# clayjohn/godot-volumetric-cloud-demo-v2

Hardware: AMD Instinct MI355X
Metric: Mrays/s + hemisphere fps, 2048x1024 @ 128x6 steps, 1/2/4/8 MI355X (higher is better)
Workload: dtype f32

## Files before the change

__graft_entry__.py:

```python
import os
import subprocess
import sys

ROOT = os.path.dirname(os.path.abspath(__file__))
PKG = os.path.join(ROOT, "godot-volumetric-cloud-demo-v2_amd")
if ROOT not in sys.path:
    sys.path.insert(0, ROOT)


def build():
    env = dict(os.environ)
    env.setdefault("PYTORCH_ROCM_ARCH", "gfx950")
    subprocess.check_call(["make", "-C", os.path.join(PKG, "csrc"), "-s", "ARCH=gfx950"], env=env)
    subprocess.check_call(["make", "-C", os.path.join(ROOT, "oracle"), "-s"])
    subprocess.check_call(["make", "-C", os.path.join(ROOT, "tests", "hostsim"), "-s"])
    subprocess.check_call(["make", "-C", os.path.join(ROOT, "tests", "satwalk"), "-s"])
    subprocess.check_call(["make", "-C", os.path.join(ROOT, "tests", "tilewalk"), "-s"])
    subprocess.check_call(["make", "-C", os.path.join(ROOT, "tests", "radiance_host"), "-s"])
    subprocess.check_call(["make", "-C", os.path.join(ROOT, "tests", "tlut_host"), "-s"])
    subprocess.check_call(["make", "-C", os.path.join(ROOT, "tests", "owners_host"), "-s"])
    subprocess.check_call(["make", "-C", os.path.join(ROOT, "tests", "lut_reuse_host"), "-s"])
    subprocess.check_call(["make", "-C", os.path.join(ROOT, "tests", "frame_ring_host"), "-s"])
    subprocess.check_call(["make", "-C", os.path.join(ROOT, "tests", "noise_set_host"), "-s"])
    subprocess.check_call(["make", "-C", os.path.join(ROOT, "tests", "mip_args_host"), "-s"])
    subprocess.check_call(["make", "-C", os.path.join(ROOT, "tests", "shadow_host"), "-s"])
    subprocess.check_call(["make", "-C", os.path.join(ROOT, "tests", "aerial_host"), "-s"])
    subprocess.check_call(["make", "-C", os.path.join(ROOT, "tests", "shafts_host"), "-s"])
    subprocess.check_call(["make", "-C", os.path.join(ROOT, "tests", "cloud_aerial_host"), "-s"])
    subprocess.check_call(["make", "-C", os.path.join(ROOT, "tests", "rays_host"), "-s"])
    subprocess.check_call(["make", "-C", os.path.join(ROOT, "gdext"), "-s"])
    subprocess.call(["make", "-C", os.path.join(PKG, "csrc"), "-s", "census", "ARCH=gfx950"], env=env)
    import gvcd_amd

    L = gvcd_amd.lib()
    assert L.csky_abi_version() == gvcd_amd._lib.ABI_VERSION
    if os.path.isdir("/root/reference/cloud_sky"):
        subprocess.check_call([sys.executable, os.path.join(ROOT, "oracle", "glsl_exec", "make_glsl_fixtures.py"), "--compile-only"], stdout=subprocess.DEVNULL)
    return None


def smoke():
    import numpy as np

    import gvcd_amd
# ... 52 lines not shown
```

godot-volumetric-cloud-demo-v2_amd/csrc/cloud_core.h:

```cpp
#pragma once
#include "csky_common.h"

namespace csky {

#if defined(__HIP_DEVICE_COMPILE__)
CSKY_HD float fast_rcp(float x) { return __builtin_amdgcn_rcpf(x); }
CSKY_HD float fast_exp2(float x) { return __builtin_amdgcn_exp2f(x); }
CSKY_HD float fast_log2(float x) { return __builtin_amdgcn_logf(x); }
#define CSKY_WAVE_ALL(x) (__all(x) != 0)
#else
CSKY_HD float fast_rcp(float x) { return 1.0f / x; }
CSKY_HD float fast_exp2(float x) { return exp2f(x); }
CSKY_HD float fast_log2(float x) { return log2f(x); }
#define CSKY_WAVE_ALL(x) (x)
#endif
CSKY_HD float fast_exp(float x) { return fast_exp2(x * 1.44269504088896f); }
CSKY_HD float fast_pow(float x, float y) { return fast_exp2(y * fast_log2(x)); }

#ifndef CSKY_PRIO_MATH
#define CSKY_PRIO_MATH 1
#endif
#if defined(__HIP_DEVICE_COMPILE__) && CSKY_PRIO_MATH > 0
#define CSKY_PRIO(n) __builtin_amdgcn_s_setprio(n)
#else
// ... 314 lines not shown
        const uint32_t sh2 = (uint32_t)(5 - lvl);
        const uint16_t* __restrict__ d = T.detail_lds + detail_level_offset(lvl);
        const uint32_t r00 = (((uint32_t)z0 << sh2) | (uint32_t)y0) << sh2, r10 = (((uint32_t)z0 << sh2) | (uint32_t)y1) << sh2;
        const uint32_t r01 = (((uint32_t)z1 << sh2) | (uint32_t)y0) << sh2, r11 = (((uint32_t)z1 << sh2) | (uint32_t)y1) << sh2;
        const uint32_t p00 = (uint32_t)d[r00 + x0] | ((uint32_t)d[r00 + x1] << 16), p10 = (uint32_t)d[r10 + x0] | ((uint32_t)d[r10 + x1] << 16);
        const uint32_t p01 = (uint32_t)d[r01 + x0] | ((uint32_t)d[r01 + x1] << 16), p11 = (uint32_t)d[r11 + x0] | ((uint32_t)d[r11 + x1] << 16);
        return lerpf(lerpf(lerp_h2(p00, ax), lerp_h2(p10, ax), ay), lerpf(lerp_h2(p01, ax), lerp_h2(p11, ax), ay), az) * (1.0f / (8.0f * 255.0f));
    }
    const uint32_t sh = (uint32_t)(5 - lvl), idx = detail_level_offset(lvl) + ((((((uint32_t)z0 << sh) | (uint32_t)y0) << sh)) | (uint32_t)x0);
    const uint4 q = *reinterpret_cast<const uint4*>(reinterpret_cast<const char*>(T.detail) + (idx << 4));
    return fmaf(az, fmaf(ay, lerp_h(q.w, ax), lerp_h(q.z, ax)), fmaf(ay, lerp_h(q.y, ax), lerp_h(q.x, ax))) * (1.0f / (8.0f * 255.0f));
}

CSKY_HD float height_fraction(float r) { return sat((r - SKY_B_RADIUS) * (1.0f / (SKY_T_RADIUS - SKY_B_RADIUS))); }

CSKY_HD float density_height_gradient(const FrameConsts& fc, float hf, float ct) {
    const float c = ct;
    constexpr float K = 1.0f / 255.0f;
    float gx, d1, gz, d2;
    if (fc.ct_mode == 1) {
        gx = 0.03f + c * (-0.02f * K); d1 = (0.3375f - 0.03f) + c * ((-0.275f + 0.02f) * K); gz = 0.18f + c * (0.6f * K); d2 = (0.25f - 0.18f) + c * ((0.75f - 0.6f) * K);
    } else if (fc.ct_mode == 2) {
        gx = 0.02f + c * 0.0f; d1 = (0.05f - 0.02f) + c * (0.3f * K); gz = 0.09f + c * (0.78f * K); d2 = (0.11f - 0.09f) + c * ((1.03f - 0.78f) * K);
    } else {
        const bool hi = ct >= 127.5f;
        gx = (hi ? 0.03f : 0.02f) + c * (hi ? -0.02f * K : 0.0f);
        d1 = (hi ? 0.3375f - 0.03f : 0.05f - 0.02f) + c * (hi ? (-0.275f + 0.02f) * K : 0.3f * K);
        gz = (hi ? 0.18f : 0.09f) + c * (hi ? 0.6f * K : 0.78f * K);
        d2 = (hi ? 0.25f - 0.18f : 0.11f - 0.09f) + c * (hi ? (0.75f - 0.6f) * K : (1.03f - 0.78f) * K);
    }
    const float r = fast_rcp(d1 * d2);
    const float t = sat((hf - gx) * (r * d2)) - sat((hf - gz) * (r * d1));
    return t * t * (3.0f - 2.0f * t);
}

template <class TS>
CSKY_HD float density(const TS& T, const FrameConsts& fc, float px, float py, float pz, float hf, float wr, float wb,
                      int lod_shape, int lod_detail) {
    const float wc = fc.cov255 * wb;
    const float g = density_height_gradient(fc, hf, wr);
    const float omw = 1.0f - wc;
    if (!(g > omw)) return 0.0f;
    float qx, qy, qz, sx, sy, sz;
    shape_coord(fc, px, py, pz, qx, qy, qz, sx, sy, sz);
#ifdef CSKY_BRICK_BOUND
    if (lod_shape == 0) {
        int bx, by, bz; float fx_, fy_, fz_;
        split_coord(sx * 128.0f - 0.5f, bx, fx_); split_coord(sy * 128.0f - 0.5f, by, fy_); split_coord(sz * 128.0f - 0.5f, bz, fz_);
        const uint32_t bi = ((((uint32_t)bz & 127u) >> 3) << 8) | ((((uint32_t)by & 127u) >> 3) << 4) | (((uint32_t)bx & 127u) >> 3);
        const float bm = T.brick[bi];
        if (!(bm * g > omw)) return 0.0f;
    }
#endif
    float nr, fbm;
    shape_tap(T, lod_shape, sx, sy, sz, nr, fbm);
// ... 2 lines not shown
    float num = (nr + omf) * g - omw * den1;
    if (!(num > 0.0f)) return 0.0f;
#ifdef CSKY_RESTORE_WC_FACTOR
    num = num * (wc * fast_rcp(1.0f - omw));
#endif
    detail_coord(fc, qx, qy, qz, sx, sy, sz);
    float hfbm = detail_tap(T, lod_detail, sx, sy, sz);
    CSKY_STAGE(3);
    const float k = sat(hf * 4.0f);
    hfbm = hfbm + k * (1.0f - 2.0f * hfbm);
    const float hm = hfbm * 0.4f * hf, den2 = 1.0f - hm;
    const float base = (num - hm * den1) * fast_rcp(den1 * den2);
    return fast_pow(sat(base), (1.0f - hf) * 0.8f + 0.5f);
}

template <class TS>
CSKY_HD float sample_density(const TS& T, const FrameConsts& fc, float px, float py, float pz, float hf, float wx, float wy,
                             int lod_shape, int lod_detail) {
    CSKY_STAGE(0);
    if (!(hf > fc.hf_lo && hf < fc.hf_hi)) return 0.0f;
    float wsx, wsy, wr, wb;
    weather_coord(px, pz, wx, wy, wsx, wsy);
    weather_tap_ts(T, wsx, wsy, wr, wb);
    CSKY_STAGE(1);
    return density(T, fc, px, py, pz, hf, wr, wb, lod_shape, lod_detail);
}

#if CSKY_SHAPE_POLY == 3
template <bool EAGER_DETAIL = true, bool SMALL_TABLE = false, class TS>
CSKY_HD float sample_density_eager(const TS& T, const FrameConsts& fc, float px, float py, float pz, float hf, float wx, float wy,
                                   int lod_shape, int lod_detail) {
    if constexpr (TS::cell32) return sample_density(T, fc, px, py, pz, hf, wx, wy, lod_shape, lod_detail);
    float d = 0.0f;
    if (hf > fc.hf_lo && hf < fc.hf_hi) {
        CSKY_PRIO(0);
        float wsx, wsy;
        weather_coord(px, pz, wx, wy, wsx, wsy);
        int wix, wiy; float wax, way;
        split_coord(wsx * 512.0f - 0.5f, wix, wax); split_coord(wsy * 512.0f - 0.5f, wiy, way);
        const uint4 wq = *reinterpret_cast<const uint4*>(reinterpret_cast<const char*>(T.weather) + (((((uint32_t)(wiy & 511)) << 9) | (uint32_t)(wix & 511)) << 4));
        float qx, qy, qz, sx, sy, sz;
        shape_coord(fc, px, py, pz, qx, qy, qz, sx, sy, sz);
        const int sn = SHAPE_N >> lod_shape, sm = sn - 1;
        const float sfn = pow2f(7 - lod_shape);
        int six, siy, siz; float sax, say, saz;
        split_coord(sx * sfn - 0.5f, six, sax); split_coord(sy * sfn - 0.5f, siy, say); split_coord(sz * sfn - 0.5f, siz, saz);
        const uint32_t ssh = (uint32_t)(7 - lod_shape);
        const uint32_t sidx = shape_level_offset(lod_shape) + shape_cell_offset((uint32_t)(six & sm), (uint32_t)(siy & sm), (uint32_t)(siz & sm), ssh);
        const uint4* __restrict__ sp = reinterpret_cast<const uint4*>(reinterpret_cast<const char*>(T.shape) + (sidx << 5));
        const uint4 tr = sp[0], tf = sp[1];
        float dsx, dsy, dsz;
        detail_coord(fc, qx, qy, qz, dsx, dsy, dsz);
        const bool tap = EAGER_DETAIL && lod_detail != 5;
        uint4 dq;
        float dax, day, daz;
        if (tap) {
            const int dn = DETAIL_N >> lod_detail, dm = dn - 1;
            const float dfn = pow2f(5 - lod_detail);
            int dix, diy, diz;
            split_coord(dsx * dfn - 0.5f, dix, dax); split_coord(dsy * dfn - 0.5f, diy, day); split_coord(dsz * dfn - 0.5f, diz, daz);
            const uint32_t dsh = (uint32_t)(5 - lod_detail);
            const uint32_t dlo = detail_level_offset(lod_detail), dcell = (((((uint32_t)(diz & dm)) << dsh) | (uint32_t)(diy & dm)) << dsh) | (uint32_t)(dix & dm);
            const uint32_t didx = dlo + dcell;
            if constexpr (SMALL_TABLE) {
                static_assert(TS::small_detail && EAGER_DETAIL, "the table belongs to the persistent form's light march");
                const uint32_t dfirst = lod_detail == TS::SMALL_DETAIL_FIRST ? 0u : detail_level_offset(TS::SMALL_DETAIL_FIRST + 1) - detail_level_offset(TS::SMALL_DETAIL_FIRST);
                const SmallDetailCell c = T.det_small[dfirst + dcell];
                dq.x = c.x; dq.y = c.y; dq.z = c.z; dq.w = c.w;
            } else {
                dq = *reinterpret_cast<const uint4*>(reinterpret_cast<const char*>(T.detail) + (didx << 4));
            }
        }
        CSKY_PRIO(CSKY_PRIO_MATH);
        const float wr = fmaf(way, lerp_h(wq.y, wax), lerp_h(wq.x, wax));
        const float wb = fmaf(way, lerp_h(wq.w, wax), lerp_h(wq.z, wax));
        const float wc = fc.cov255 * wb;
        const float g = density_height_gradient(fc, hf, wr);
        const float omw = 1.0f - wc;
        if (g > omw) {
            const float nr = fmaf(saz, fmaf(say, lerp_h(tr.w, sax), lerp_h(tr.z, sax)), fmaf(say, lerp_h(tr.y, sax), lerp_h(tr.x, sax))) * (1.0f / 255.0f);
            const float fbm = fmaf(saz, fmaf(say, lerp_h(tf.w, sax), lerp_h(tf.z, sax)), fmaf(say, lerp_h(tf.y, sax), lerp_h(tf.x, sax))) * (1.0f / (8.0f * 255.0f));
            const float omf = 1.0f - fbm, den1 = 1.0f + omf;
            float num = (nr + omf) * g - omw * den1;
            if (num > 0.0f) {
#ifdef CSKY_RESTORE_WC_FACTOR
                num = num * (wc * fast_rcp(1.0f - omw));
#endif
                float hfbm;
                if (tap) hfbm = fmaf(daz, fmaf(day, lerp_h(dq.w, dax), lerp_h(dq.z, dax)), fmaf(day, lerp_h(dq.y, dax), lerp_h(dq.x, dax))) * (1.0f / (8.0f * 255.0f));
                else if (EAGER_DETAIL) hfbm = T.detail_lod5;
                else hfbm = detail_tap(T, lod_detail, dsx, dsy, dsz);
                const float k = sat(hf * 4.0f);
                hfbm = hfbm + k * (1.0f - 2.0f * hfbm);
                const float hm = hfbm * 0.4f * hf, den2 = 1.0f - hm;
                const float base = (num - hm * den1) * fast_rcp(den1 * den2);
                d = fast_pow(sat(base), (1.0f - hf) * 0.8f + 0.5f);
            }
        }
    }
    return d;
}
#else
template <bool EAGER_DETAIL = true, bool SMALL_TABLE = false, class TS>
CSKY_HD float sample_density_eager(const TS& T, const FrameConsts& fc, float px, float py, float pz, float hf, float wx, float wy,
                                   int lod_shape, int lod_detail) {
    return sample_density(T, fc, px, py, pz, hf, wx, wy, lod_shape, lod_detail);
}
#endif

CSKY_HD float henyey_greenstein(float c, float g) {
    const float x = 1.0f + g * g - 2.0f * g * c;
    return 0.0795774715459f * (1.0f - g * g) / (x * sqrtf(x));
}

CSKY_HD void shade_terms(const FrameConsts& fc, float phase, float t, float hf, float dt, float cd, float& Dr, float& Dg, float& Db, float& q) {
    const float lss = (SKY_T_RADIUS - SKY_B_RADIUS) / 64.0f;
    const float nd = -fc.density;
    const float beers = fast_exp(nd * cd * lss * 3.0f);
    const float powder = 1.0f - beers * beers;
    const float bt = 2.0f * beers * powder;
    const float sm = hf * hf * (3.0f - 2.0f * hf);
// ... 89 lines not shown
```

godot-volumetric-cloud-demo-v2_amd/csrc/cloud_kernels.hip:

```cpp
#include <hip/hip_runtime.h>
#include "kernels.h"
#include "cloud_core.h"
#include "order_core.h"
#pragma clang fp contract(off)

namespace csky {

constexpr int QCAP = 96;
constexpr int QSTEPS = 48;
constexpr int Q_FLOATS = 5 * QCAP + 7 * QCAP + 3 * QSTEPS;

__device__ __forceinline__ void wave_lds_fence() {
    __builtin_amdgcn_fence(__ATOMIC_RELEASE, "wavefront");
    __builtin_amdgcn_wave_barrier();
    __builtin_amdgcn_fence(__ATOMIC_ACQUIRE, "wavefront");
}

__device__ __forceinline__ float ray_phase(const FrameConsts& fc, const Ray& ray) {
    float phase = 0.0f;
    if (ray.above) {
        const float ct = fc.ldir[0] * ray.dx + fc.ldir[1] * ray.dy + fc.ldir[2] * ray.dz;
        phase = fmaxf(fmaxf(henyey_greenstein(ct, 0.6f), henyey_greenstein(ct, fc.hg_g2)), henyey_greenstein(ct, -0.2f));
    }
    return phase;
// ... 93 lines not shown
            if (!__any(live)) break;
        }
    }
    o.r = Lr; o.g = Lg; o.b = Lb; o.a = sat(alpha); o.t = Tr;
    return o;
}

constexpr int CQ_CAP = 128;
constexpr int CQ_STEPS = 66;
constexpr int CQ_FLOATS = 5 * CQ_CAP + CQ_CAP / 4 + 3 * CQ_STEPS + 2 + 128 + 320;

#ifndef CSKY_EAGER_LIGHT
#define CSKY_EAGER_LIGHT 1
#endif
#if CSKY_EAGER_LIGHT
#define CSKY_LIGHT_SAMPLE sample_density_eager<true>
#else
#define CSKY_LIGHT_SAMPLE sample_density
#endif
#ifndef CSKY_EAGER_PRIMARY
#define CSKY_EAGER_PRIMARY 0
#endif
#if CSKY_EAGER_PRIMARY == 1
#define CSKY_PRIMARY_SAMPLE sample_density_eager<false>
#elif CSKY_EAGER_PRIMARY == 2
#define CSKY_PRIMARY_SAMPLE sample_density_eager<true>
#else
#define CSKY_PRIMARY_SAMPLE sample_density
#endif
template <class TS, class Late>
__device__ __forceinline__ void light_march_terms(const TS& T, const FrameConsts& fc, const int ls, const float nd, float ex, float ey, float ez, Late&& late,
                                                  float& Dr, float& Dg, float& Db, float& rq, float& dt) {
    float lx = ex, ly = ey, lz = ez, cd = 0.0f;
#if CSKY_EAGER_LIGHT
    constexpr int JS = TS::small_detail ? 3 : 6;
#else
    constexpr int JS = 6;
#endif
#pragma unroll 1
    for (int j = 0; j < JS; j++) {
        if (j >= ls) break;
        advance(lx, ly, lz, fc.linc[j][0], fc.linc[j][1], fc.linc[j][2]);
        const float lhf = height_fraction(length3_shell(lx, ly, lz));
        cd += CSKY_LIGHT_SAMPLE(T, fc, lx, ly, lz, lhf, fc.wpos_x, fc.wpos_y, j > 2 ? j - 2 : 0, j);
    }
#if CSKY_EAGER_LIGHT
    if constexpr (TS::small_detail) {
#pragma unroll 1
        for (int j = JS; j < 6; j++) {
            if (j >= ls) break;
            advance(lx, ly, lz, fc.linc[j][0], fc.linc[j][1], fc.linc[j][2]);
            const float lhf = height_fraction(length3_shell(lx, ly, lz));
            cd += sample_density_eager<true, true>(T, fc, lx, ly, lz, lhf, fc.wpos_x, fc.wpos_y, j - 2, j);
        }
    }
#endif
    {
        lx = ex; ly = ey; lz = ez;
        advance(lx, ly, lz, fc.ldist[0], fc.ldist[1], fc.ldist[2]);
        const float lhf = height_fraction(length3_shell(lx, ly, lz));
        const float ld = CSKY_LIGHT_SAMPLE(T, fc, lx, ly, lz, lhf, 0.0f, 0.0f, 3, 5);
        cd += fast_pow(ld, (1.0f - lhf) * 0.8f + 0.5f);
    }
    float et, ehf, ess, eph;
    late(et, ehf, ess, eph);
    dt = fast_exp(nd * et * ess);
    shade_terms(fc, eph, et, ehf, dt, cd, Dr, Dg, Db, rq);
}

template <bool WHOLE, bool TALLY, class TS>
__device__ __forceinline__ MarchOut march_compact(const TS& T, const FrameConsts& fc, Ray ray, float* __restrict__ q, int step_begin, int step_end) {
    constexpr bool SAT = WHOLE && !TS::cell32;
    constexpr bool DEAD = SAT && !TALLY;
    float* __restrict__ ev_px = q;
    float* __restrict__ ev_py = q + CQ_CAP;
    float* __restrict__ ev_pz = q + 2 * CQ_CAP;
    float* __restrict__ ev_t = q + 3 * CQ_CAP;
    float* __restrict__ ev_hf = q + 4 * CQ_CAP;
    unsigned char* __restrict__ ev_owner = reinterpret_cast<unsigned char*>(q + 5 * CQ_CAP);
    unsigned* __restrict__ st_lo = reinterpret_cast<unsigned*>(q + 5 * CQ_CAP + CQ_CAP / 4);
    unsigned* __restrict__ st_hi = st_lo + CQ_STEPS;
    unsigned* __restrict__ st_base = st_hi + CQ_STEPS;

    MarchOut o; o.r = o.g = o.b = o.a = 0.0f; o.t = 1.0f; o.incloud = 0;
    const int lane = threadIdx.x & 63;
// ... 10 lines not shown
    float* __restrict__ ray_ss = reinterpret_cast<float*>(tally + 2);
    float* __restrict__ ray_ph = ray_ss + 64;
    ray_ss[lane] = ray.ss; ray_ph[lane] = phase;
    float* __restrict__ acc = ray_ph + 64;
    acc[lane] = 1.0f; acc[64 + lane] = 0.0f; acc[128 + lane] = 0.0f; acc[192 + lane] = 0.0f; acc[256 + lane] = 0.0f;
    if (__builtin_amdgcn_ballot_w64(live) == 0ull) return o;
    for (int i = 0; i < step_begin; i++) advance(px, py, pz, ray.sx, ray.sy, ray.sz);
    int end = step_end;
    for (int i = step_begin;;) {
        if (i < end) {
            float t, hf;
            bool have = false, below_top = false;
            if (live) {
                advance(px, py, pz, ray.sx, ray.sy, ray.sz);
                hf = height_fraction(length3_shell(px, py, pz));
                t = CSKY_PRIMARY_SAMPLE(T, fc, px, py, pz, hf, fc.wpos_x, fc.wpos_y, 0, 0);
                have = t > 0.0f;
                below_top = !(hf >= fc.hf_hi);
            }
            if constexpr (SAT && TALLY) {
                skipped += (unsigned)__popcll(__builtin_amdgcn_ballot_w64(have && latched));
                have = have && !latched;
            }
            if ((i & 3) == 3 && __builtin_amdgcn_ballot_w64(below_top) == 0ull) end = i + 1;
            const unsigned long long m = __builtin_amdgcn_ballot_w64(have);
            if (m != 0ull) {
                const int slot = count + (int)__builtin_amdgcn_mbcnt_hi((unsigned)(m >> 32), __builtin_amdgcn_mbcnt_lo((unsigned)m, 0u));
                if (have) { ev_px[slot] = px; ev_py[slot] = py; ev_pz[slot] = pz; ev_t[slot] = t; ev_hf[slot] = hf; ev_owner[slot] = (unsigned char)lane; }
                if (lane == 0) { st_lo[cs] = (unsigned)m; st_hi[cs] = (unsigned)(m >> 32); st_base[cs] = (unsigned)count; }
                count += __popcll(m);
                cs++;
            }
            i++;
        }
        const bool last = i >= end;
        if (count == 0) { if (last) break; continue; }
        if (count < 64 && !last) continue;
        wave_lds_fence();
        const int n = count < 64 ? count : 64;
        unsigned long long carry = 0ull;
        if constexpr (TALLY) { if (lane == 0) tally[0] += (unsigned)n; }
        if (lane < n) {
            float Dr, Dg, Db, rq, dt;
            light_march_terms(T, fc, ls, nd, ev_px[lane], ev_py[lane], ev_pz[lane],
                              [&](float& et, float& ehf, float& ess, float& eph) { et = ev_t[lane]; ehf = ev_hf[lane]; const int ow = ev_owner[lane]; ess = ray_ss[ow]; eph = ray_ph[ow]; }, Dr, Dg, Db, rq, dt);
            ev_px[lane] = Dr; ev_py[lane] = Dg; ev_pz[lane] = Db; ev_t[lane] = rq; ev_hf[lane] = dt;
        }
        wave_lds_fence();
        float Tr = acc[lane], alpha = acc[64 + lane], Lr = acc[128 + lane], Lg = acc[192 + lane], Lb = acc[256 + lane];
        for (int s = 0; s < cs; s++) {
            const unsigned lo = (unsigned)__builtin_amdgcn_readfirstlane((int)st_lo[s]), hi = (unsigned)__builtin_amdgcn_readfirstlane((int)st_hi[s]);
            const bool mine = __builtin_amdgcn_inverse_ballot_w64(((unsigned long long)hi << 32) | lo);
            const int slot = (int)st_base[s] + (int)__builtin_amdgcn_mbcnt_hi(hi, __builtin_amdgcn_mbcnt_lo(lo, 0u));
            if (mine && slot < n) {
                composite_sample(ev_hf[slot], ev_t[slot], ev_px[slot], ev_py[slot], ev_pz[slot], Tr, alpha, Lr, Lg, Lb);
            }
            if (s == cs - 1) carry = __builtin_amdgcn_ballot_w64(mine && slot >= n);
        }
        if constexpr (DEAD) {
// ... 198 lines not shown
        store_pixel(out, G, pix.gx, pix.gy, pix.lr, o.r, o.g, o.b, o.a);
    }
    if (stats || wg_cost) {
        unsigned ic = o.incloud, ab = ray.above ? 1u : 0u;
        for (int off = 32; off > 0; off >>= 1) { ic += __shfl_down(ic, off); ab += __shfl_down(ab, off); }
        if (lane == 0) {
            if (stats) { atomicAdd(&stats[0], (unsigned long long)ic); atomicAdd(&stats[1], (unsigned long long)ab); }
            if (wg_cost) atomicAdd(&wg_cost[logical], ic + 16u * ab);
        }
    }
}

#ifndef CSKY_COMPACT_WAVES
#define CSKY_COMPACT_WAVES 7
#endif
template <int VARIANT, int SEG, class TS = TexSet, bool TALLY = true>
__device__ __forceinline__ void render_block(TS T, const FrameConsts* __restrict__ fcp, const RenderGeom& G, const uint32_t logical, const uint32_t rec,
                                             uint2* __restrict__ out, unsigned long long* __restrict__ stats, uint32_t* __restrict__ wg_cost, const int tile_of_wave = -1) {
    constexpr int BW = 32 / SEG;
    const int tiles_x = (G.tile_w + BW - 1) / BW;
    const int local_rows = G.n_bands * G.band_rows;
    const int slab = (int)logical / tiles_x, bx = (int)logical - slab * tiles_x;
    const int wave = threadIdx.x >> 6, lane = threadIdx.x & 63;
    const int tile = tile_of_wave >= 0 ? tile_of_wave : wave / SEG, seg = tile_of_wave >= 0 ? 0 : wave - tile * SEG;
    const int gx = bx * BW + tile * 8 + (lane & 7);
    const int lr = slab * 8 + (lane >> 3);
    const bool valid = gx < G.tile_w && lr < local_rows;
    const int band = lr / G.band_rows, rib = lr - band * G.band_rows;
    const int gy = (G.first_band + band * G.band_stride) * G.band_rows + rib;

    const FrameConsts& fc = *fcp;
    T.detail_lds = nullptr;
    Ray ray = ray_setup(fc, valid ? gx : 0, valid ? gy : 0);
    if (!valid) ray.above = false;
    MarchOut o;
    if constexpr (VARIANT == 0) {
        static_assert(SEG == 1, "the lock-step reference variant marches whole rays");
        o = march(T, fc, ray);
    } else {
        __shared__ float lds[4][VARIANT == 3 ? CQ_FLOATS : Q_FLOATS];
        const int s0 = (fc.primary_steps * seg) / SEG, s1 = (fc.primary_steps * (seg + 1)) / SEG;
        if constexpr (VARIANT == 3) o = march_compact<SEG == 1, TALLY>(T, fc, ray, &lds[wave][0], s0, s1);
        else o = march_queue(T, fc, ray, &lds[wave][0], s0, s1);
        if constexpr (SEG > 1) {
            __shared__ float comb[4][5][64];
            comb[wave][0][lane] = o.r; comb[wave][1][lane] = o.g; comb[wave][2][lane] = o.b; comb[wave][3][lane] = o.t; comb[wave][4][lane] = o.a;
            __syncthreads();
            if (seg == 0) {
                float Tr = o.t, na = 1.0f - o.a;
#pragma unroll
                for (int s = 1; s < SEG; s++) {
                    const int w = tile * SEG + s;
                    o.r += Tr * comb[w][0][lane]; o.g += Tr * comb[w][1][lane]; o.b += Tr * comb[w][2][lane];
                    Tr *= comb[w][3][lane]; na *= 1.0f - comb[w][4][lane];
                }
                o.a = sat(1.0f - na); o.t = Tr;
            }
// ... 10 lines not shown
            if (stats) { atomicAdd(&stats[0], (unsigned long long)ic); atomicAdd(&stats[1], (unsigned long long)ab); }
            if (wg_cost) atomicAdd(&wg_cost[logical], ic + 16u * ab);
        }
    }
    }
}

template <int VARIANT, int SEG, class TS = TexSet, bool TALLY = true>
__global__ __launch_bounds__(256, VARIANT == 3 ? CSKY_COMPACT_WAVES : 7) void clouds_kernel(TS T, const FrameConsts* __restrict__ fcp, RenderGeom G, const uint32_t* __restrict__ order,
                                                     uint2* __restrict__ out, unsigned long long* __restrict__ stats, uint32_t* __restrict__ wg_cost) {
    const uint32_t logical = order[blockIdx.x];
    if (logical == 0xffffffffu) return;
    render_block<VARIANT, SEG, TS, TALLY>(T, fcp, G, logical, blockIdx.x, out, stats, wg_cost);
}

template <int VARIANT, bool TALLY = true>
__global__ __launch_bounds__(256, VARIANT == 3 ? CSKY_COMPACT_WAVES : 7) void clouds_kernel_persistent(TexSet T, const FrameConsts* __restrict__ fcp, RenderGeom G,
        const uint32_t* __restrict__ order, const uint32_t n_items, uint32_t* __restrict__ heads, uint2* __restrict__ out, unsigned long long* __restrict__ stats,
        uint32_t* __restrict__ wg_cost) {
    unsigned xcc;
    asm volatile("s_getreg_b32 %0, hwreg(HW_REG_XCC_ID)" : "=s"(xcc));
    xcc &= 7u;
    __shared__ uint32_t ticket, slot_ready[2], slot_reads[2], slot_entry[2], slot_rec[2];
    if (threadIdx.x == 0) { ticket = 0; slot_ready[0] = slot_ready[1] = 0; slot_reads[0] = slot_reads[1] = 0; }
    static_assert(VARIANT == 3, "the persistent form exists for the compact march only: its light march is the one that reads the table");
    __shared__ __attribute__((aligned(16))) uint4 det_small[TexSetSmallDetail::SMALL_DETAIL_CELLS];
    if (threadIdx.x < (unsigned)TexSetSmallDetail::SMALL_DETAIL_CELLS) det_small[threadIdx.x] = T.detail[detail_level_offset(TexSetSmallDetail::SMALL_DETAIL_FIRST) + threadIdx.x];
    __syncthreads();
    const bool lane0 = (threadIdx.x & 63) == 0;
    for (;;) {
        uint32_t tv = 0;
// ... 28 lines not shown
            }
            logical = (uint32_t)__builtin_amdgcn_readfirstlane((int)slot_entry[sl]);
            rec = (uint32_t)__builtin_amdgcn_readfirstlane((int)slot_rec[sl]);
            if (lane0) __hip_atomic_fetch_add(&slot_reads[sl], 1u, __ATOMIC_RELEASE, __HIP_MEMORY_SCOPE_WORKGROUP);
        }
        if (logical == 0xfffffffeu) {
            if (lane0 && atomicAdd(&heads[8], 1u) == gridDim.x * 4u - 1u) {
                for (unsigned k = 0; k < 9u; k++) atomicExch(&heads[k], 0u);
            }
            return;
        }
        if (logical != 0xffffffffu) {
            TexSetSmallDetail Ts;
            static_cast<TexSet&>(Ts) = T;
            Ts.det_small = (SmallDetailTable)det_small;
            render_block<VARIANT, 1, TexSetSmallDetail, TALLY>(Ts, fcp, G, logical, rec, out, stats, wg_cost, tile);
        }
    }
}


__global__ __launch_bounds__(256) void lpt_hist_kernel(const uint32_t* __restrict__ cost, int n, int shift, uint32_t* __restrict__ hist) {
    const int i = blockIdx.x * 256 + threadIdx.x;
    if (i < n) atomicAdd(&hist[lpt_bucket(cost[i], shift)], 1u);
}
__global__ __launch_bounds__(LPT_BUCKETS) void lpt_scan_kernel(uint32_t* __restrict__ hist, uint32_t* __restrict__ offsets) {
    __shared__ uint32_t sh[LPT_BUCKETS];
    const int t = threadIdx.x;
    const uint32_t own = hist[t];
    hist[t] = 0u;
    sh[t] = own;
// ... 54 lines not shown
    const size_t i = (size_t)blockIdx.x * 256 + threadIdx.x;
    if (i < n) out[i] = sqrt_shell(in[i]);
}
hipError_t launch_sqrt_shell(const float* d_in, float* d_out, size_t n, hipStream_t s) {
    if (n == 0) return hipSuccess;
    sqrt_shell_kernel<<<(unsigned)((n + 255) / 256), 256, 0, s>>>(d_in, d_out, n);
    return hipGetLastError();
}

static const char* const kVariantNames[] = {"lockstep", "queue", "queue-lds", "compact"};
int cloud_resident_workgroups_per_cu() { return CSKY_COMPACT_WAVES; }
int cloud_variant_count() { return (int)(sizeof(kVariantNames) / sizeof(kVariantNames[0])); }
const char* cloud_variant_name(int v) { return (v >= 0 && v < cloud_variant_count()) ? kVariantNames[v] : nullptr; }

hipError_t launch_clouds(int variant, int seg, const TexSet& t, const FrameConsts* d_fc, const RenderGeom& g, const uint32_t* d_order, int grid,
                         uint2* d_out, unsigned long long* d_stats, uint32_t* d_wg_cost, hipStream_t s, uint32_t* d_heads, int resident, const TexSet32* t32, bool census_lean) {
    if (grid <= 0) return hipSuccess;
    const bool tally = (d_stats != nullptr || d_wg_cost != nullptr) && !census_lean;
    if (t32) {
        if (variant != 3 || seg != 1) return hipErrorInvalidValue;
        clouds_kernel<3, 1, TexSet32><<<grid, 256, 0, s>>>(*t32, d_fc, g, d_order, d_out, d_stats, d_wg_cost);
        return hipGetLastError();
    }
    if (d_heads && variant == 3 && seg == 1) {
        if (tally) clouds_kernel_persistent<3, true><<<grid < resident ? grid : resident, 256, 0, s>>>(t, d_fc, g, d_order, (uint32_t)grid, d_heads, d_out, d_stats, d_wg_cost);
        else clouds_kernel_persistent<3, false><<<grid < resident ? grid : resident, 256, 0, s>>>(t, d_fc, g, d_order, (uint32_t)grid, d_heads, d_out, d_stats, d_wg_cost);
        return hipGetLastError();
    }
    if (variant == 0 && seg == 1) clouds_kernel<0, 1><<<grid, 256, 0, s>>>(t, d_fc, g, d_order, d_out, d_stats, d_wg_cost);
    else if (variant == 1 && seg == 1) clouds_kernel<1, 1><<<grid, 256, 0, s>>>(t, d_fc, g, d_order, d_out, d_stats, d_wg_cost);
    else if (variant == 1 && seg == 2) clouds_kernel<1, 2><<<grid, 256, 0, s>>>(t, d_fc, g, d_order, d_out, d_stats, d_wg_cost);
    else if (variant == 1 && seg == 4) clouds_kernel<1, 4><<<grid, 256, 0, s>>>(t, d_fc, g, d_order, d_out, d_stats, d_wg_cost);
    else if (variant == 3 && seg == 1 && tally) clouds_kernel<3, 1, TexSet, true><<<grid, 256, 0, s>>>(t, d_fc, g, d_order, d_out, d_stats, d_wg_cost);
    else if (variant == 3 && seg == 1) clouds_kernel<3, 1, TexSet, false><<<grid, 256, 0, s>>>(t, d_fc, g, d_order, d_out, d_stats, d_wg_cost);
    else if (variant == 3 && seg == 2) clouds_kernel<3, 2><<<grid, 256, 0, s>>>(t, d_fc, g, d_order, d_out, d_stats, d_wg_cost);
    else if (variant == 3 && seg == 4) clouds_kernel<3, 4><<<grid, 256, 0, s>>>(t, d_fc, g, d_order, d_out, d_stats, d_wg_cost);
    else if ((variant == 1 || variant == 3) && seg == 5) {
        hipError_t e = hipFuncSetAttribute(reinterpret_cast<const void*>(&clouds_kernel_interleaved<0>), hipFuncAttributeMaxDynamicSharedMemorySize,
                                           (int)(IL_BLOCK_FLOATS * sizeof(float)));
        if (e != hipSuccess) return e;
        clouds_kernel_interleaved<0><<<grid, 256, IL_BLOCK_FLOATS * sizeof(float), s>>>(t, d_fc, g, d_order, d_out, d_stats, d_wg_cost);
// ... 57 lines not shown
```

godot-volumetric-cloud-demo-v2_amd/csrc/clouds_launch.cpp:

```cpp
#include <cstring>
#include "context.h"
#include "launch_policy.h"
#include "order_core.h"

namespace csky {

TexSet texset(const csky_ctx* c) {
    const NoiseSet& n = c->noise;
    TexSet t;
#ifdef CSKY_BRICK_BOUND
    t.brick = n.d_brick;
#endif
    t.shape = n.d_shape; t.detail = n.d_detail; t.weather = n.d_weather; t.sky = c->lut.cur_f(); t.sky_w = c->lut.aw; t.sky_h = c->lut.ah; t.detail_lod5 = n.st.detail_lod5(); t.detail_h = n.d_detail_h; t.detail_lds = nullptr;
    return t;
}

TexSet32 texset32(const csky_ctx* c) {
    TexSet32 t;
    static_cast<TexSet&>(t) = texset(c);
    t.shape32 = c->noise.d_shape32; t.detail32 = c->noise.d_detail32; t.weather32 = c->noise.d_weather32;
    return t;
}

namespace {

int ensure_order(csky_ctx* c, int slot, int mode, int tiles_x, int slabs, hipStream_t s) {
    const int grid = static_order_grid(mode, tiles_x, slabs);
    const OrderKey key = order_key(tiles_x, slabs, mode, grid);
    FrameSlot& f = c->ring.slot[slot];
    if (f.order_st.hit(f.order != nullptr, key)) return CSKY_OK;
    if (f.order.count() < (size_t)grid) { int rc; if ((rc = c->ring.grow_order_tables(c, (size_t)grid))) return rc; }
    HIPCHK(c, launch_static_order(mode, tiles_x, slabs, grid, f.order, s));
    f.order_st.written(key);
    return CSKY_OK;
}

int frame_setup(csky_ctx* c, const CloudParams& cp, hipStream_t s) {
    const ExactRejects rej = c->noise.st.rejects(cp.cloud_coverage, c->use_window);
    int f, rc; if ((rc = c->ring.next_slot(c, c->stream, f))) return rc;
    const SetupArgs sa = {c->primary_steps, c->light_steps, c->early_eps, rej.hf_lo, rej.hf_hi, rej.ct_mode, c->use_window ? 1 : 0};
    const SkyLut& l = c->lut;
    if (l.st.own_taps())
        HIPCHK(c, launch_frame_setup_taps(cp, l.st.sun, c->d_trans_f, c->tw, c->th, l.st.w, l.st.h, sa, c->ring.slot[f].fc, c->stream, c->tlut));
    else
        HIPCHK(c, launch_frame_setup(cp, l.cur_f(), l.aw, l.ah, sa, c->ring.slot[f].fc, c->stream));
    return c->ring.setup_enqueued(c, f, c->stream, s);
}

}

int check_bands(csky_ctx* c, const csky_bands* b, int tile_w) {
    if (tile_w < 1 || !b || b->band_rows < 1 || b->n_bands < 0 || b->first_band < 0 || b->band_stride < 1)
        return fail(c, CSKY_ERR_INVALID, "render_clouds: bad tile/bands description");
    return CSKY_OK;
}
// ... 21 lines not shown
    if (c->noise.st.cell32()) { t32 = texset32(c); t32p = &t32; }
    const Event* kt = nullptr;
    if (c->kt.on && (rc = c->kt.next_pair(c, kt))) return rc;
    if ((rc = ensure_order(c, slot, pl.static_mode, tiles_x, slabs, s))) return rc;
    const uint32_t* order = ring.slot[slot].order;
    int grid = ring.slot[slot].order_st.grid();
    uint32_t* cost = nullptr;
    if (pl.feedback) {
        if ((rc = ring.reserve_feedback(c, (size_t)(grid > nblocks ? grid : nblocks)))) return rc;
        cost = ring.cost(slot);
        const FeedbackKey fkey = feedback_key(g.tile_w, g.band_rows, g.first_band, g.band_stride, g.n_bands, cp.texture_size, cp.update_position, pl.mode, pl.static_mode, pl.seg);
        if (ring.slot[slot].feedback.begin(fkey)) { order = ring.feedback_order(slot); grid = nblocks; }
    }
    if (kt) HIPCHK(c, hipEventRecord(kt[0], s));
    {
        const hipError_t le = launch_clouds(pl.variant, pl.seg, texset(c), ring.fc(), g, order, grid, d_out, d_stats, cost, s, heads, c->resident_wgs, t32p, c->census_lean);
        if (le != hipSuccess) { if (heads) (void)hipMemsetAsync(heads, 0, 16 * sizeof(uint32_t), s); return fail(c, CSKY_ERR_HIP, "cloud kernel launch failed: %s", hipGetErrorString(le)); }
    }
    if (kt) HIPCHK(c, hipEventRecord(kt[1], s));
    if (pl.feedback) {
        HIPCHK(c, launch_lpt_order(cost, nblocks, lpt_shift(c->primary_steps), ring.sort_scratch(slot), ring.feedback_order(slot), s));
        ring.slot[slot].feedback.sort_enqueued();
    }
    return ring.march_enqueued(c, slot, s);
}

}
```

godot-volumetric-cloud-demo-v2_amd/csrc/kernels.h:

```cpp
#pragma once
#include <hip/hip_runtime_api.h>
#include "csky_common.h"
#include "composite_core.h"
#include "noise_core.h"

namespace csky {

hipError_t launch_transmittance(int w, int h, uint16_t* d_half, float4* d_float, hipStream_t s, int tlut = 0);
hipError_t launch_sky_lut(int w, int h, const float sun[3], const float4* d_trans, int tw, int th, uint16_t* d_half,
                          float4* d_float, hipStream_t s, int tlut = 0);
hipError_t launch_sky_lut_rows(int w, int h, int row0, int row_stride, const float sun[3], const float4* d_trans, int tw, int th, uint2* d_rows, float4* d_whole_f,
                               hipStream_t s, int tlut = 0);
hipError_t launch_composite(const CompositeArgs& a, uint2* d_out, hipStream_t s, int tlut = 0);
struct SetupArgs {
    int primary_steps, light_steps;
    float early_eps, hf_lo, hf_hi;
    int ct_mode, sat_skip;
};
hipError_t launch_frame_setup(const CloudParams& p, const float4* d_sky, int sw, int sh, const SetupArgs& a, FrameConsts* d_fc, hipStream_t s);
hipError_t launch_frame_setup_taps(const CloudParams& p, const float sun[3], const float4* d_trans, int tw, int th, int sw, int sh, const SetupArgs& a, FrameConsts* d_fc,
                                   hipStream_t s, int tlut = 0);

hipError_t launch_shape_noise(uint32_t seed, int n, const ShapeNoiseParams& P, uint32_t* d_out, hipStream_t s);
hipError_t launch_detail_noise(uint32_t seed, int n, uint8_t* d_out, hipStream_t s);
hipError_t launch_mip_chain(uint8_t* d_chain, int n, int ch, int levels, hipStream_t s);
hipError_t launch_bake(const uint8_t* d_large_chain, const uint8_t* d_small_chain, const uint8_t* d_weather, ShapeTexel* d_shape, uint4* d_detail, uint16_t* d_detail_h,
                       uint4* d_weather_out, unsigned long long* d_inexact, int* d_range, hipStream_t s);
hipError_t launch_bake32(const uint8_t* d_large_chain, const uint8_t* d_small_chain, const uint8_t* d_weather, float4* d_shape32, float4* d_detail32, float4* d_weather32, hipStream_t s);

hipError_t launch_clouds(int variant, int seg, const TexSet& t, const FrameConsts* d_fc, const RenderGeom& g, const uint32_t* d_order, int grid,
                         uint2* d_out, unsigned long long* d_stats, uint32_t* d_wg_cost, hipStream_t s, uint32_t* d_heads = nullptr, int resident = 0,
                         const TexSet32* t32 = nullptr, bool census_lean = false);
int cloud_resident_workgroups_per_cu();
int cloud_variant_count();
const char* cloud_variant_name(int v);
hipError_t launch_lpt_order(uint32_t* d_cost, int n, int shift, uint32_t* d_scratch, uint32_t* d_order, hipStream_t s);
hipError_t launch_static_order(int mode, int tiles_x, int slabs, int grid, uint32_t* d_order, hipStream_t s);
hipError_t launch_interleave_bands(const void* d_gathered, size_t member_stride_bytes, int members, size_t band_bytes, int total_bands, void* d_frame, hipStream_t s);
hipError_t launch_sqrt_shell(const float* d_in, float* d_out, size_t n, hipStream_t s);
struct RaysGeom;
hipError_t launch_clouds_rays(const TexSet& t, const TexSet32* t32, const FrameConsts* d_fc, const RaysGeom& g, const float* d_dirs, uint2* d_out, hipStream_t s);

struct ShadowConsts;
hipError_t launch_cloud_shadow(const TexSet& t, const TexSet32* t32, const FrameConsts& fc, const ShadowConsts& sc, uint16_t* d_out, hipStream_t s);

struct AerialGeom;
hipError_t launch_aerial(const AerialGeom& g, const float4* d_trans, int tw, int th, uint2* d_out, hipStream_t s, int tlut = 0);
// ... 21 lines not shown
```

Measured before the change: 1582.

## Specialize persistent cloud kernel on cloud-type mode and straighten light march

Result: faster. 1640, median of 6 (+3.7%).

```diff
diff --git a/__graft_entry__.py b/__graft_entry__.py
--- a/__graft_entry__.py
+++ b/__graft_entry__.py
@@ -28,6 +28,7 @@
     subprocess.check_call(["make", "-C", os.path.join(ROOT, "tests", "shafts_host"), "-s"])
     subprocess.check_call(["make", "-C", os.path.join(ROOT, "tests", "cloud_aerial_host"), "-s"])
     subprocess.check_call(["make", "-C", os.path.join(ROOT, "tests", "rays_host"), "-s"])
+    subprocess.check_call(["make", "-C", os.path.join(ROOT, "tests", "gradient_host"), "-s"])
     subprocess.check_call(["make", "-C", os.path.join(ROOT, "gdext"), "-s"])
     subprocess.call(["make", "-C", os.path.join(PKG, "csrc"), "-s", "census", "ARCH=gfx950"], env=env)
     import gvcd_amd
diff --git a/godot-volumetric-cloud-demo-v2_amd/csrc/cloud_core.h b/godot-volumetric-cloud-demo-v2_amd/csrc/cloud_core.h
--- a/godot-volumetric-cloud-demo-v2_amd/csrc/cloud_core.h
+++ b/godot-volumetric-cloud-demo-v2_amd/csrc/cloud_core.h
@@ -352,13 +352,15 @@
 
 CSKY_HD float height_fraction(float r) { return sat((r - SKY_B_RADIUS) * (1.0f / (SKY_T_RADIUS - SKY_B_RADIUS))); }
 
+template <int CT = 0>
 CSKY_HD float density_height_gradient(const FrameConsts& fc, float hf, float ct) {
+    static_assert(CT >= 0 && CT <= 2, "cloud-type mode: 0 generic, 1 every texel >= 0.5, 2 every texel < 0.5");
     const float c = ct;
     constexpr float K = 1.0f / 255.0f;
     float gx, d1, gz, d2;
-    if (fc.ct_mode == 1) {
+    if (CT == 1 || (CT == 0 && fc.ct_mode == 1)) {
         gx = 0.03f + c * (-0.02f * K); d1 = (0.3375f - 0.03f) + c * ((-0.275f + 0.02f) * K); gz = 0.18f + c * (0.6f * K); d2 = (0.25f - 0.18f) + c * ((0.75f - 0.6f) * K);
-    } else if (fc.ct_mode == 2) {
+    } else if (CT == 2 || (CT == 0 && fc.ct_mode == 2)) {
         gx = 0.02f + c * 0.0f; d1 = (0.05f - 0.02f) + c * (0.3f * K); gz = 0.09f + c * (0.78f * K); d2 = (0.11f - 0.09f) + c * ((1.03f - 0.78f) * K);
     } else {
         const bool hi = ct >= 127.5f;
@@ -372,11 +374,11 @@
     return t * t * (3.0f - 2.0f * t);
 }
 
-template <class TS>
+template <int CT = 0, class TS>
 CSKY_HD float density(const TS& T, const FrameConsts& fc, float px, float py, float pz, float hf, float wr, float wb,
                       int lod_shape, int lod_detail) {
     const float wc = fc.cov255 * wb;
-    const float g = density_height_gradient(fc, hf, wr);
+    const float g = density_height_gradient<CT>(fc, hf, wr);
     const float omw = 1.0f - wc;
     if (!(g > omw)) return 0.0f;
     float qx, qy, qz, sx, sy, sz;
@@ -409,7 +411,7 @@
     return fast_pow(sat(base), (1.0f - hf) * 0.8f + 0.5f);
 }
 
-template <class TS>
+template <int CT = 0, class TS>
 CSKY_HD float sample_density(const TS& T, const FrameConsts& fc, float px, float py, float pz, float hf, float wx, float wy,
                              int lod_shape, int lod_detail) {
     CSKY_STAGE(0);
@@ -418,14 +420,20 @@
     weather_coord(px, pz, wx, wy, wsx, wsy);
     weather_tap_ts(T, wsx, wsy, wr, wb);
     CSKY_STAGE(1);
-    return density(T, fc, px, py, pz, hf, wr, wb, lod_shape, lod_detail);
+    return density<CT>(T, fc, px, py, pz, hf, wr, wb, lod_shape, lod_detail);
 }
 
 #if CSKY_SHAPE_POLY == 3
-template <bool EAGER_DETAIL = true, bool SMALL_TABLE = false, class TS>
+CSKY_HD uint32_t level_offset_scalar(uint32_t off) {
+#if defined(__HIP_DEVICE_COMPILE__)
+    asm("" : "+s"(off));
+#endif
+    return off;
+}
+template <bool EAGER_DETAIL = true, bool SMALL_TABLE = false, int CT = 0, class TS>
 CSKY_HD float sample_density_eager(const TS& T, const FrameConsts& fc, float px, float py, float pz, float hf, float wx, float wy,
                                    int lod_shape, int lod_detail) {
-    if constexpr (TS::cell32) return sample_density(T, fc, px, py, pz, hf, wx, wy, lod_shape, lod_detail);
+    if constexpr (TS::cell32) return sample_density<CT>(T, fc, px, py, pz, hf, wx, wy, lod_shape, lod_detail);
     float d = 0.0f;
     if (hf > fc.hf_lo && hf < fc.hf_hi) {
         CSKY_PRIO(0);
@@ -441,7 +449,8 @@
         int six, siy, siz; float sax, say, saz;
         split_coord(sx * sfn - 0.5f, six, sax); split_coord(sy * sfn - 0.5f, siy, say); split_coord(sz * sfn - 0.5f, siz, saz);
         const uint32_t ssh = (uint32_t)(7 - lod_shape);
-        const uint32_t sidx = shape_level_offset(lod_shape) + shape_cell_offset((uint32_t)(six & sm), (uint32_t)(siy & sm), (uint32_t)(siz & sm), ssh);
+        const uint32_t slo = CT != 0 ? level_offset_scalar(shape_level_offset(lod_shape)) : shape_level_offset(lod_shape);
+        const uint32_t sidx = slo + shape_cell_offset((uint32_t)(six & sm), (uint32_t)(siy & sm), (uint32_t)(siz & sm), ssh);
         const uint4* __restrict__ sp = reinterpret_cast<const uint4*>(reinterpret_cast<const char*>(T.shape) + (sidx << 5));
         const uint4 tr = sp[0], tf = sp[1];
         float dsx, dsy, dsz;
@@ -455,7 +464,7 @@
             int dix, diy, diz;
             split_coord(dsx * dfn - 0.5f, dix, dax); split_coord(dsy * dfn - 0.5f, diy, day); split_coord(dsz * dfn - 0.5f, diz, daz);
             const uint32_t dsh = (uint32_t)(5 - lod_detail);
-            const uint32_t dlo = detail_level_offset(lod_detail), dcell = (((((uint32_t)(diz & dm)) << dsh) | (uint32_t)(diy & dm)) << dsh) | (uint32_t)(dix & dm);
+            const uint32_t dlo = (CT != 0 && !SMALL_TABLE) ? level_offset_scalar(detail_level_offset(lod_detail)) : detail_level_offset(lod_detail), dcell = (((((uint32_t)(diz & dm)) << dsh) | (uint32_t)(diy & dm)) << dsh) | (uint32_t)(dix & dm);
             const uint32_t didx = dlo + dcell;
             if constexpr (SMALL_TABLE) {
                 static_assert(TS::small_detail && EAGER_DETAIL, "the table belongs to the persistent form's light march");
@@ -470,7 +479,7 @@
         const float wr = fmaf(way, lerp_h(wq.y, wax), lerp_h(wq.x, wax));
         const float wb = fmaf(way, lerp_h(wq.w, wax), lerp_h(wq.z, wax));
         const float wc = fc.cov255 * wb;
-        const float g = density_height_gradient(fc, hf, wr);
+        const float g = density_height_gradient<CT>(fc, hf, wr);
         const float omw = 1.0f - wc;
         if (g > omw) {
             const float nr = fmaf(saz, fmaf(say, lerp_h(tr.w, sax), lerp_h(tr.z, sax)), fmaf(say, lerp_h(tr.y, sax), lerp_h(tr.x, sax))) * (1.0f / 255.0f);
@@ -496,10 +505,10 @@
     return d;
 }
 #else
-template <bool EAGER_DETAIL = true, bool SMALL_TABLE = false, class TS>
+template <bool EAGER_DETAIL = true, bool SMALL_TABLE = false, int CT = 0, class TS>
 CSKY_HD float sample_density_eager(const TS& T, const FrameConsts& fc, float px, float py, float pz, float hf, float wx, float wy,
                                    int lod_shape, int lod_detail) {
-    return sample_density(T, fc, px, py, pz, hf, wx, wy, lod_shape, lod_detail);
+    return sample_density<CT>(T, fc, px, py, pz, hf, wx, wy, lod_shape, lod_detail);
 }
 #endif
 
diff --git a/godot-volumetric-cloud-demo-v2_amd/csrc/cloud_kernels.hip b/godot-volumetric-cloud-demo-v2_amd/csrc/cloud_kernels.hip
--- a/godot-volumetric-cloud-demo-v2_amd/csrc/cloud_kernels.hip
+++ b/godot-volumetric-cloud-demo-v2_amd/csrc/cloud_kernels.hip
@@ -2,6 +2,7 @@
 #include "kernels.h"
 #include "cloud_core.h"
 #include "order_core.h"
+#include <type_traits>
 #pragma clang fp contract(off)
 
 namespace csky {
@@ -131,44 +132,65 @@
 #define CSKY_EAGER_LIGHT 1
 #endif
 #if CSKY_EAGER_LIGHT
-#define CSKY_LIGHT_SAMPLE sample_density_eager<true>
+#define CSKY_LIGHT_SAMPLE(CT) sample_density_eager<true, false, CT>
 #else
-#define CSKY_LIGHT_SAMPLE sample_density
+#define CSKY_LIGHT_SAMPLE(CT) sample_density<CT>
 #endif
 #ifndef CSKY_EAGER_PRIMARY
 #define CSKY_EAGER_PRIMARY 0
 #endif
 #if CSKY_EAGER_PRIMARY == 1
-#define CSKY_PRIMARY_SAMPLE sample_density_eager<false>
+#define CSKY_PRIMARY_SAMPLE(CT) sample_density_eager<false, false, CT>
 #elif CSKY_EAGER_PRIMARY == 2
-#define CSKY_PRIMARY_SAMPLE sample_density_eager<true>
+#define CSKY_PRIMARY_SAMPLE(CT) sample_density_eager<true, false, CT>
 #else
-#define CSKY_PRIMARY_SAMPLE sample_density
+#define CSKY_PRIMARY_SAMPLE(CT) sample_density<CT>
 #endif
-template <class TS, class Late>
+#ifndef CSKY_LIGHT_STRAIGHT
+#define CSKY_LIGHT_STRAIGHT 1
+#endif
+#if CSKY_EAGER_LIGHT
+template <int CT, int J, class TS>
+__device__ __forceinline__ void light_samples_from(const TS& T, const FrameConsts& fc, const int ls, float& lx, float& ly, float& lz, float& cd) {
+    if constexpr (J < 6) {
+        if (J >= ls) return;
+        advance(lx, ly, lz, fc.linc[J][0], fc.linc[J][1], fc.linc[J][2]);
+        const float lhf = height_fraction(length3_shell(lx, ly, lz));
+        cd += sample_density_eager<true, (J > 2), CT>(T, fc, lx, ly, lz, lhf, fc.wpos_x, fc.wpos_y, J > 2 ? J - 2 : 0, J);
+        light_samples_from<CT, J + 1>(T, fc, ls, lx, ly, lz, cd);
+    }
+}
+#endif
+template <int CT = 0, class TS, class Late>
 __device__ __forceinline__ void light_march_terms(const TS& T, const FrameConsts& fc, const int ls, const float nd, float ex, float ey, float ez, Late&& late,
                                                   float& Dr, float& Dg, float& Db, float& rq, float& dt) {
     float lx = ex, ly = ey, lz = ez, cd = 0.0f;
 #if CSKY_EAGER_LIGHT
     constexpr int JS = TS::small_detail ? 3 : 6;
+    constexpr bool STRAIGHT = CSKY_LIGHT_STRAIGHT && TS::small_detail && CT != 0;
 #else
     constexpr int JS = 6;
+    constexpr bool STRAIGHT = false;
 #endif
+    if constexpr (!STRAIGHT) {
 #pragma unroll 1
-    for (int j = 0; j < JS; j++) {
-        if (j >= ls) break;
-        advance(lx, ly, lz, fc.linc[j][0], fc.linc[j][1], fc.linc[j][2]);
-        const float lhf = height_fraction(length3_shell(lx, ly, lz));
-        cd += CSKY_LIGHT_SAMPLE(T, fc, lx, ly, lz, lhf, fc.wpos_x, fc.wpos_y, j > 2 ? j - 2 : 0, j);
+        for (int j = 0; j < JS; j++) {
+            if (j >= ls) break;
+            advance(lx, ly, lz, fc.linc[j][0], fc.linc[j][1], fc.linc[j][2]);
+            const float lhf = height_fraction(length3_shell(lx, ly, lz));
+            cd += CSKY_LIGHT_SAMPLE(CT)(T, fc, lx, ly, lz, lhf, fc.wpos_x, fc.wpos_y, j > 2 ? j - 2 : 0, j);
+        }
     }
 #if CSKY_EAGER_LIGHT
-    if constexpr (TS::small_detail) {
+    if constexpr (STRAIGHT) {
+        light_samples_from<CT, 0>(T, fc, ls, lx, ly, lz, cd);
+    } else if constexpr (TS::small_detail) {
 #pragma unroll 1
         for (int j = JS; j < 6; j++) {
             if (j >= ls) break;
             advance(lx, ly, lz, fc.linc[j][0], fc.linc[j][1], fc.linc[j][2]);
             const float lhf = height_fraction(length3_shell(lx, ly, lz));
-            cd += sample_density_eager<true, true>(T, fc, lx, ly, lz, lhf, fc.wpos_x, fc.wpos_y, j - 2, j);
+            cd += sample_density_eager<true, true, CT>(T, fc, lx, ly, lz, lhf, fc.wpos_x, fc.wpos_y, j - 2, j);
         }
     }
 #endif
@@ -176,7 +198,7 @@
         lx = ex; ly = ey; lz = ez;
         advance(lx, ly, lz, fc.ldist[0], fc.ldist[1], fc.ldist[2]);
         const float lhf = height_fraction(length3_shell(lx, ly, lz));
-        const float ld = CSKY_LIGHT_SAMPLE(T, fc, lx, ly, lz, lhf, 0.0f, 0.0f, 3, 5);
+        const float ld = CSKY_LIGHT_SAMPLE(CT)(T, fc, lx, ly, lz, lhf, 0.0f, 0.0f, 3, 5);
         cd += fast_pow(ld, (1.0f - lhf) * 0.8f + 0.5f);
     }
     float et, ehf, ess, eph;
@@ -185,7 +207,7 @@
     shade_terms(fc, eph, et, ehf, dt, cd, Dr, Dg, Db, rq);
 }
 
-template <bool WHOLE, bool TALLY, class TS>
+template <bool WHOLE, bool TALLY, int CT = 0, class TS>
 __device__ __forceinline__ MarchOut march_compact(const TS& T, const FrameConsts& fc, Ray ray, float* __restrict__ q, int step_begin, int step_end) {
     constexpr bool SAT = WHOLE && !TS::cell32;
     constexpr bool DEAD = SAT && !TALLY;
@@ -226,7 +248,7 @@
             if (live) {
                 advance(px, py, pz, ray.sx, ray.sy, ray.sz);
                 hf = height_fraction(length3_shell(px, py, pz));
-                t = CSKY_PRIMARY_SAMPLE(T, fc, px, py, pz, hf, fc.wpos_x, fc.wpos_y, 0, 0);
+                t = CSKY_PRIMARY_SAMPLE(CT)(T, fc, px, py, pz, hf, fc.wpos_x, fc.wpos_y, 0, 0);
                 have = t > 0.0f;
                 below_top = !(hf >= fc.hf_hi);
             }
@@ -254,7 +276,7 @@
         if constexpr (TALLY) { if (lane == 0) tally[0] += (unsigned)n; }
         if (lane < n) {
             float Dr, Dg, Db, rq, dt;
-            light_march_terms(T, fc, ls, nd, ev_px[lane], ev_py[lane], ev_pz[lane],
+            light_march_terms<CT>(T, fc, ls, nd, ev_px[lane], ev_py[lane], ev_pz[lane],
                               [&](float& et, float& ehf, float& ess, float& eph) { et = ev_t[lane]; ehf = ev_hf[lane]; const int ow = ev_owner[lane]; ess = ray_ss[ow]; eph = ray_ph[ow]; }, Dr, Dg, Db, rq, dt);
             ev_px[lane] = Dr; ev_py[lane] = Dg; ev_pz[lane] = Db; ev_t[lane] = rq; ev_hf[lane] = dt;
         }
@@ -483,7 +505,7 @@
 #ifndef CSKY_COMPACT_WAVES
 #define CSKY_COMPACT_WAVES 7
 #endif
-template <int VARIANT, int SEG, class TS = TexSet, bool TALLY = true>
+template <int VARIANT, int SEG, class TS = TexSet, bool TALLY = true, int CT = 0>
 __device__ __forceinline__ void render_block(TS T, const FrameConsts* __restrict__ fcp, const RenderGeom& G, const uint32_t logical, const uint32_t rec,
                                              uint2* __restrict__ out, unsigned long long* __restrict__ stats, uint32_t* __restrict__ wg_cost, const int tile_of_wave = -1) {
     constexpr int BW = 32 / SEG;
@@ -509,7 +531,7 @@
     } else {
         __shared__ float lds[4][VARIANT == 3 ? CQ_FLOATS : Q_FLOATS];
         const int s0 = (fc.primary_steps * seg) / SEG, s1 = (fc.primary_steps * (seg + 1)) / SEG;
-        if constexpr (VARIANT == 3) o = march_compact<SEG == 1, TALLY>(T, fc, ray, &lds[wave][0], s0, s1);
+        if constexpr (VARIANT == 3) o = march_compact<SEG == 1, TALLY, CT>(T, fc, ray, &lds[wave][0], s0, s1);
         else o = march_queue(T, fc, ray, &lds[wave][0], s0, s1);
         if constexpr (SEG > 1) {
             __shared__ float comb[4][5][64];
@@ -550,7 +572,7 @@
     render_block<VARIANT, SEG, TS, TALLY>(T, fcp, G, logical, blockIdx.x, out, stats, wg_cost);
 }
 
-template <int VARIANT, bool TALLY = true>
+template <int VARIANT, bool TALLY = true, int CT = 0>
 __global__ __launch_bounds__(256, VARIANT == 3 ? CSKY_COMPACT_WAVES : 7) void clouds_kernel_persistent(TexSet T, const FrameConsts* __restrict__ fcp, RenderGeom G,
         const uint32_t* __restrict__ order, const uint32_t n_items, uint32_t* __restrict__ heads, uint2* __restrict__ out, unsigned long long* __restrict__ stats,
         uint32_t* __restrict__ wg_cost) {
@@ -609,7 +631,7 @@
             TexSetSmallDetail Ts;
             static_cast<TexSet&>(Ts) = T;
             Ts.det_small = (SmallDetailTable)det_small;
-            render_block<VARIANT, 1, TexSetSmallDetail, TALLY>(Ts, fcp, G, logical, rec, out, stats, wg_cost, tile);
+            render_block<VARIANT, 1, TexSetSmallDetail, TALLY, CT>(Ts, fcp, G, logical, rec, out, stats, wg_cost, tile);
         }
     }
 }
@@ -694,8 +716,10 @@
 const char* cloud_variant_name(int v) { return (v >= 0 && v < cloud_variant_count()) ? kVariantNames[v] : nullptr; }
 
 hipError_t launch_clouds(int variant, int seg, const TexSet& t, const FrameConsts* d_fc, const RenderGeom& g, const uint32_t* d_order, int grid,
-                         uint2* d_out, unsigned long long* d_stats, uint32_t* d_wg_cost, hipStream_t s, uint32_t* d_heads, int resident, const TexSet32* t32, bool census_lean) {
+                         uint2* d_out, unsigned long long* d_stats, uint32_t* d_wg_cost, hipStream_t s, uint32_t* d_heads, int resident, const TexSet32* t32, bool census_lean,
+                         int ct_mode) {
     if (grid <= 0) return hipSuccess;
+    if (ct_mode < 0 || ct_mode > 2) return hipErrorInvalidValue;
     const bool tally = (d_stats != nullptr || d_wg_cost != nullptr) && !census_lean;
     if (t32) {
         if (variant != 3 || seg != 1) return hipErrorInvalidValue;
@@ -703,8 +727,16 @@
         return hipGetLastError();
     }
     if (d_heads && variant == 3 && seg == 1) {
-        if (tally) clouds_kernel_persistent<3, true><<<grid < resident ? grid : resident, 256, 0, s>>>(t, d_fc, g, d_order, (uint32_t)grid, d_heads, d_out, d_stats, d_wg_cost);
-        else clouds_kernel_persistent<3, false><<<grid < resident ? grid : resident, 256, 0, s>>>(t, d_fc, g, d_order, (uint32_t)grid, d_heads, d_out, d_stats, d_wg_cost);
+        const unsigned n = (unsigned)(grid < resident ? grid : resident);
+        const auto go = [&](auto tl, auto ct) {
+            clouds_kernel_persistent<3, decltype(tl)::value, decltype(ct)::value><<<n, 256, 0, s>>>(t, d_fc, g, d_order, (uint32_t)grid, d_heads, d_out, d_stats, d_wg_cost);
+        };
+        const auto with_mode = [&](auto tl) {
+            if (ct_mode == 1) go(tl, std::integral_constant<int, 1>());
+            else if (ct_mode == 2) go(tl, std::integral_constant<int, 2>());
+            else go(tl, std::integral_constant<int, 0>());
+        };
+        if (tally) with_mode(std::true_type()); else with_mode(std::false_type());
         return hipGetLastError();
     }
     if (variant == 0 && seg == 1) clouds_kernel<0, 1><<<grid, 256, 0, s>>>(t, d_fc, g, d_order, d_out, d_stats, d_wg_cost);
diff --git a/godot-volumetric-cloud-demo-v2_amd/csrc/clouds_launch.cpp b/godot-volumetric-cloud-demo-v2_amd/csrc/clouds_launch.cpp
--- a/godot-volumetric-cloud-demo-v2_amd/csrc/clouds_launch.cpp
+++ b/godot-volumetric-cloud-demo-v2_amd/csrc/clouds_launch.cpp
@@ -35,10 +35,14 @@
     return CSKY_OK;
 }
 
+SetupArgs setup_args(csky_ctx* c, const CloudParams& cp) {
+    const ExactRejects rej = c->noise.st.rejects(cp.cloud_coverage, c->use_window);
+    return {c->primary_steps, c->light_steps, c->early_eps, rej.hf_lo, rej.hf_hi, rej.ct_mode, c->use_window ? 1 : 0};
+}
+
 int frame_setup(csky_ctx* c, const CloudParams& cp, hipStream_t s) {
-    const ExactRejects rej = c->noise.st.rejects(cp.cloud_coverage, c->use_window);
+    const SetupArgs sa = setup_args(c, cp);
     int f, rc; if ((rc = c->ring.next_slot(c, c->stream, f))) return rc;
-    const SetupArgs sa = {c->primary_steps, c->light_steps, c->early_eps, rej.hf_lo, rej.hf_hi, rej.ct_mode, c->use_window ? 1 : 0};
     const SkyLut& l = c->lut;
     if (l.st.own_taps())
         HIPCHK(c, launch_frame_setup_taps(cp, l.st.sun, c->d_trans_f, c->tw, c->th, l.st.w, l.st.h, sa, c->ring.slot[f].fc, c->stream, c->tlut));
@@ -90,7 +94,8 @@
     }
     if (kt) HIPCHK(c, hipEventRecord(kt[0], s));
     {
-        const hipError_t le = launch_clouds(pl.variant, pl.seg, texset(c), ring.fc(), g, order, grid, d_out, d_stats, cost, s, heads, c->resident_wgs, t32p, c->census_lean);
+        const hipError_t le = launch_clouds(pl.variant, pl.seg, texset(c), ring.fc(), g, order, grid, d_out, d_stats, cost, s, heads, c->resident_wgs, t32p, c->census_lean,
+                                                setup_args(c, cp).ct_mode);
         if (le != hipSuccess) { if (heads) (void)hipMemsetAsync(heads, 0, 16 * sizeof(uint32_t), s); return fail(c, CSKY_ERR_HIP, "cloud kernel launch failed: %s", hipGetErrorString(le)); }
     }
     if (kt) HIPCHK(c, hipEventRecord(kt[1], s));
diff --git a/godot-volumetric-cloud-demo-v2_amd/csrc/kernels.h b/godot-volumetric-cloud-demo-v2_amd/csrc/kernels.h
--- a/godot-volumetric-cloud-demo-v2_amd/csrc/kernels.h
+++ b/godot-volumetric-cloud-demo-v2_amd/csrc/kernels.h
@@ -30,7 +30,8 @@
 
 hipError_t launch_clouds(int variant, int seg, const TexSet& t, const FrameConsts* d_fc, const RenderGeom& g, const uint32_t* d_order, int grid,
                          uint2* d_out, unsigned long long* d_stats, uint32_t* d_wg_cost, hipStream_t s, uint32_t* d_heads = nullptr, int resident = 0,
-                         const TexSet32* t32 = nullptr, bool census_lean = false);
+                         const TexSet32* t32 = nullptr, bool census_lean = false,
+                         int ct_mode = 0);
 int cloud_resident_workgroups_per_cu();
 int cloud_variant_count();
 const char* cloud_variant_name(int v);
```
